# JamesBrofos/Stein

Measured on AMD Instinct MI355X. Metric: SVGD particle-updates/sec, higher is better.
Workload: dtype f32; 1 GPU; C3 bayesian-logreg-shaped synthetic block n=16384 d=256 fp32 (roofline config); n=16384, d=256, rows_per_rank=16384, optimizer=adagrad lr=1e-3 alpha=0.9, parallelism=single GPU

## Files before the change

stein_amd/csrc/stein_x3.hip:

```cpp

#include "stein_x3.h"

#include <stdlib.h>

#include "stein_x3_dev.h"
template <int KIND> struct SplitTraits { static constexpr int pexp = KIND == 2 ? PEXP_H2 : 0; };

#include <type_traits>

__device__ __forceinline__ int xswz(int row, int chunk) { return (chunk ^ ((row >> 2) & 3)) * 16; }

__device__ __forceinline__ u32 cvt_pk_bf16(float lo, float hi) {
  u32 r;
  asm("v_cvt_pk_bf16_f32 %0, %1, %2" : "=v"(r) : "v"(lo), "v"(hi));
  return r;
}

template <int KIND>
__device__ __forceinline__ void split_pair(float x, float y, u32 (&w)[3]) {
  if (KIND == 2) {
    w[0] = cvt_pk_f16(x, y);
    w[1] = cvt_pk_f16(f16_resid_lo(w[0], x), f16_resid_hi(w[0], y));
  } else {
    w[0] = cvt_pk_bf16(x, y);
  }
}


__device__ __forceinline__ void write_global_scales(float* __restrict__ sc, int dc, int sa, int pexp) {
  sc[4 * dc + 0] = pow2i(sa);
  sc[4 * dc + 1] = pow2i(1 - 2 * sa);
  sc[4 * dc + 2] = pow2i(-pexp);
}

__device__ __forceinline__ void make_scales_body(const u32* cmax, int dc, float* __restrict__ sc, int pexp, int enable,
                                                 u32* red) {
  const int t = threadIdx.x;
  if (t < 256) {
    u32 m = 0u;
    for (int c = t; c < dc; c += 256) {
      const u32 mg = load_fresh(cmax + c), mt = load_fresh(cmax + dc + c);
      const int sg = enable ? scale_exp(mg, 100) : 0, st = enable ? scale_exp(mt, 100) : 0;
      sc[c] = pow2i(sg);
      sc[dc + c] = pow2i(st);
      sc[2 * dc + c] = pow2i(-sg - pexp);
      sc[3 * dc + c] = pow2i(-st - pexp);
      m = max(m, mt);
    }
    red[t] = m;
  }
  __syncthreads();
  for (int o = 128; o > 0; o >>= 1) {
    if (t < o) red[t] = max(red[t], red[t + o]);
    __syncthreads();
  }
  if (t == 0) write_global_scales(sc, dc, enable ? scale_exp(red[0], 60) : 0, pexp);
}

template <typename TIN, bool V4>
__global__ __launch_bounds__(V4 ? 1024 : 256) void k_colmax(const TIN* __restrict__ X0, const TIN* __restrict__ X1, int n, int d,
                                                            u32* __restrict__ cmax0, int dc, int zbase, float* __restrict__ sc,
                                                            int pexp, HistSync* done) {
  const int z = blockIdx.z + zbase;
  constexpr int CW = V4 ? 4 : 1;
  constexpr int NW = V4 ? 16 : 4;
  __shared__ u32 red[256];
  const int t = threadIdx.x, cx = t & 63, ry = t >> 6;
  const TIN* const X[1] = {z ? X1 : X0};
  u32 m[1][CW];
  colmax_scan<TIN, V4, 1>(X, n, d, ((int)blockIdx.x * 64 + cx) * CW, (long)blockIdx.y * NW + ry, (long)gridDim.y * NW, m);
  colmax_commit<CW, 1>(m, cx, (int)blockIdx.x, d, red, cmax0 + (z ? dc : 0), dc);
  if (done) {
    __shared__ u32 s_last;
    asm volatile("s_waitcnt vmcnt(0)" ::: "memory");
    __syncthreads();
    if (t == 0) {
      const u32 id = (blockIdx.z * gridDim.y + blockIdx.y) * gridDim.x + blockIdx.x;
      s_last = tree_report_done(done->cm_leaf, &done->cm_top, id, gridDim.x * gridDim.y * gridDim.z) ? 1u : 0u;
    }
    __syncthreads();
    if (s_last) make_scales_body(cmax0, dc, sc, pexp, 1, red);
  }
}

__global__ __launch_bounds__(256) void k_make_scales(const u32* __restrict__ cmax, int dc, float* __restrict__ sc, int pexp,
                                                     int enable) {
  __shared__ u32 red[256];
  make_scales_body(cmax, dc, sc, pexp, enable, red);
}

constexpr int TP_WORDS = 64 * 32;
__device__ __forceinline__ int tp_index(int c, int p) { return c * 32 + ((((p >> 2) ^ (c >> 2)) & 7) << 2) + (p & 3); }
__device__ __forceinline__ int tp_pair(int t, int pass) { return 16 * pass + 4 * (t >> 6) + (((t >> 4) & 3) ^ ((t >> 2) & 2)); }

template <typename TIN>
__device__ __forceinline__ void load_row4(const TIN* __restrict__ X, int row, int col, int n, int d, int vec, float (&v)[4]) {
  if constexpr (std::is_same<TIN, float>::value) {
    if (vec) {
      const float4 x = (row < n && col < d) ? *reinterpret_cast<const float4*>(X + (size_t)row * d + col) : make_float4(0.f, 0.f, 0.f, 0.f);
      v[0] = x.x; v[1] = x.y; v[2] = x.z; v[3] = x.w;
      return;
    }
  }
#pragma unroll
  for (int q = 0; q < 4; ++q) v[q] = (row < n && col + q < d) ? elem_f32(X + (size_t)row * d + col + q) : 0.f;
}

template <int KIND>
__device__ __forceinline__ void tp_store(const u32 (*tile)[TP_WORDS], u16* __restrict__ Tt, long ntk_t, int dc, long nk,
                                         int row0, int col0, int t) {
  const int c = col0 + (t >> 2), j = row0 + (t & 3) * 16;
  if (c < dc && j < nk) {
    const int rowc = c & 127, ch0 = (j & 31) >> 3;
#pragma unroll
    for (int s = 0; s < KIND; ++s) {
      const uint4 w0 = *reinterpret_cast<const uint4*>(&tile[s][tp_index(t >> 2, (t & 3) * 8)]);
      const uint4 w1 = *reinterpret_cast<const uint4*>(&tile[s][tp_index(t >> 2, (t & 3) * 8 + 4)]);
      u16* base = Tt + (((size_t)(c >> 7) * ntk_t + (j >> 5)) * 3 + s) * XTILE_E;
      *reinterpret_cast<uint4*>(base + vfrag_offset(rowc, ch0)) = w0;
      *reinterpret_cast<uint4*>(base + vfrag_offset(rowc, ch0 + 1)) = w1;
    }
  }
}

template <typename TIN, int KIND, bool PRO = false>
__global__ __launch_bounds__(256) void k_split(const TIN* __restrict__ X0, const TIN* __restrict__ X1, int n, int d,
                                               u16* __restrict__ R0, long r_rows, int dk, u16* __restrict__ Tt0,
                                               u16* __restrict__ Tt1, int dc, long nk, const float* __restrict__ sc,
                                               int zbase, PrologueArgs pro, int vec) {
  if (PRO && blockIdx.z == gridDim.z - 1) {
    prologue_body<TIN>(X0, pro, (int)(blockIdx.y * gridDim.x + blockIdx.x), (int)(gridDim.x * gridDim.y));
    return;
  }
  const bool score = blockIdx.z + zbase != 0;
  if (score && ((int)blockIdx.x * 64 >= dc || (long)blockIdx.y * 64 >= nk)) return;
  const TIN* __restrict__ X = score ? X1 : X0;
  u16* __restrict__ R = score ? nullptr : R0;
  u16* __restrict__ Tt = score ? Tt1 : Tt0;
  const float* __restrict__ sc_all = sc + 4 * dc;
  const float* __restrict__ sc_col = sc + (score ? 0 : dc);
  __shared__ __attribute__((aligned(16))) u32 tile[KIND][TP_WORDS];
  const int t = threadIdx.x;
  const int row0 = blockIdx.y * 64, col0 = blockIdx.x * 64;
  const int lc = (t & 15) * 4;
  const long ntk_r = dk >> 5, ntk_t = nk >> 5;
  const float sa = (R && !PRO) ? *sc_all : 1.f;
  float scq[4];
#pragma unroll
  for (int q = 0; q < 4; ++q) scq[q] = (!PRO && Tt && col0 + lc + q < dc) ? sc_col[col0 + lc + q] : 1.f;
#pragma unroll
  for (int p = 0; p < 2; ++p) {
    const int pr = tp_pair(t, p), col = col0 + lc;
    float v[2][4];
#pragma unroll
    for (int h = 0; h < 2; ++h) {
      const int row = row0 + 2 * pr + h;
      load_row4(X, row, col, n, d, vec, v[h]);
      if (R && row < r_rows && col < dk) {
        u32 wa[3], wb[3];
        split_pair<KIND>(v[h][0] * sa, v[h][1] * sa, wa);
        split_pair<KIND>(v[h][2] * sa, v[h][3] * sa, wb);
        u16* dst = R + (((size_t)(row >> 7) * ntk_r + (col >> 5)) * 3) * XTILE_E + vfrag_offset(row & 127, (col & 31) >> 3) + (col & 7);
#pragma unroll
        for (int s = 0; s < KIND; ++s) *reinterpret_cast<uint2*>(dst + s * XTILE_E) = make_uint2(wa[s], wb[s]);
      }
    }
    if (Tt) {
#pragma unroll
      for (int q = 0; q < 4; ++q) {
        u32 w[3];
        split_pair<KIND>(v[0][q] * scq[q], v[1][q] * scq[q], w);
#pragma unroll
        for (int s = 0; s < KIND; ++s) tile[s][tp_index(lc + q, pr)] = w[s];
      }
    }
  }
  if (!Tt) return;
  __syncthreads();
  tp_store<KIND>(tile, Tt, ntk_t, dc, nk, row0, col0, t);
}

__global__ __launch_bounds__(256) void k_split_rows(const float* __restrict__ X, int n, int d, u16* __restrict__ R, long r_rows,
                                                    int dk, int dc, float* __restrict__ sc, int vec,
                                                    const u32* __restrict__ wgmax, int nwg) {
  __shared__ u32 s_wmax[4];
  const int t = threadIdx.x;
  const int row0 = blockIdx.y * 64, col = blockIdx.x * 64 + (t & 15) * 4;
  const long ntk_r = dk >> 5;
  u32 m = 0u;
  for (int i = t; i < nwg; i += 256) m = max(m, wgmax[i]);
  float v[2][2][4];
#pragma unroll
  for (int p = 0; p < 2; ++p)
#pragma unroll
    for (int h = 0; h < 2; ++h) load_row4(X, row0 + 2 * tp_pair(t, p) + h, col, n, d, vec, v[p][h]);
#pragma unroll
  for (int o = 32; o > 0; o >>= 1) m = max(m, (u32)__shfl_xor((int)m, o));
  if ((t & 63) == 0) s_wmax[t >> 6] = m;
  __syncthreads();
  const int sae = scale_exp(max(max(s_wmax[0], s_wmax[1]), max(s_wmax[2], s_wmax[3])), 60);
  const float sa = pow2i(sae);
  if (t == 0 && blockIdx.x == 0 && blockIdx.y == 0) write_global_scales(sc, dc, sae, PEXP_H2);
#pragma unroll
  for (int p = 0; p < 2; ++p)
#pragma unroll
    for (int h = 0; h < 2; ++h) {
      const int row = row0 + 2 * tp_pair(t, p) + h;
      if (row < r_rows && col < dk) {
        u32 wa[3], wb[3];
        split_pair<2>(v[p][h][0] * sa, v[p][h][1] * sa, wa);
        split_pair<2>(v[p][h][2] * sa, v[p][h][3] * sa, wb);
        u16* dst = R + (((size_t)(row >> 7) * ntk_r + (col >> 5)) * 3) * XTILE_E + vfrag_offset(row & 127, (col & 31) >> 3) + (col & 7);
#pragma unroll
        for (int s = 0; s < 2; ++s) *reinterpret_cast<uint2*>(dst + s * XTILE_E) = make_uint2(wa[s], wb[s]);
      }
    }
}

__global__ __launch_bounds__(256) void k_split_w(const float* __restrict__ T, const float* __restrict__ G, int n, int d,
                                                 u16* __restrict__ Wt, int dc, long nk, float* __restrict__ sc,
                                                 const u32* __restrict__ cmax, const float* __restrict__ h2p, int vec) {
  __shared__ __attribute__((aligned(16))) u32 tile[2][TP_WORDS];
  const int t = threadIdx.x;
  const int row0 = blockIdx.y * 64, col0 = blockIdx.x * 64;
  const int lc = (t & 15) * 4;
  const long ntk_t = nk >> 5;
  const float ih = 1.f / *h2p;
  float scq[4];
#pragma unroll
  for (int q = 0; q < 4; ++q) {
    const int c = col0 + lc + q;
    int se = 0;
    if (c < dc) se = scale_exp(__float_as_uint(__builtin_fmaf(__uint_as_float(cmax[dc + c]), ih, __uint_as_float(cmax[c]))), 100);
    scq[q] = pow2i(se);
    if (blockIdx.y == 0 && (t >> 4) == 0 && c < dc) {
      sc[c] = scq[q];
      sc[2 * dc + c] = pow2i(-se - PEXP_H2);
      const int st = scale_exp(cmax[dc + c], 100);
      sc[dc + c] = pow2i(st);
      sc[3 * dc + c] = pow2i(-st - PEXP_H2);
    }
  }
#pragma unroll
  for (int p = 0; p < 2; ++p) {
    const int pr = tp_pair(t, p), col = col0 + lc;
    float v[2][4];
#pragma unroll
    for (int h = 0; h < 2; ++h) {
      const int row = row0 + 2 * pr + h;
      float th[4], g[4];
      load_row4(T, row, col, n, d, vec, th);
      load_row4(G, row, col, n, d, vec, g);
#pragma unroll
      for (int q = 0; q < 4; ++q) v[h][q] = (row < n && col + q < d) ? __builtin_fmaf(-th[q], ih, g[q]) : 0.f;
    }
#pragma unroll
    for (int q = 0; q < 4; ++q) {
      u32 w[3];
      split_pair<2>(v[0][q] * scq[q], v[1][q] * scq[q], w);
#pragma unroll
      for (int s = 0; s < 2; ++s) tile[s][tp_index(lc + q, pr)] = w[s];
    }
  }
  __syncthreads();
  tp_store<2>(tile, Wt, ntk_t, dc, nk, row0, col0, t);
}

__device__ __forceinline__ const u16* t3_chunk_ptr(const u16* __restrict__ T3, long ntk, long grow, int c16) {
  return T3 + ((size_t)(grow >> 7) * ntk * 3) * XTILE_E + vfrag_offset((int)(grow & 127), c16);
}

template <int NP>
__device__ __forceinline__ void t3_load(const u16* __restrict__ p0, const u16* __restrict__ p1, int kt, u32x4 (&reg)[6]) {
#pragma unroll
  for (int s = 0; s < NP; ++s) {
    reg[s * 2 + 0] = *reinterpret_cast<const u32x4*>(p0 + ((size_t)kt * 3 + s) * XTILE_E);
    reg[s * 2 + 1] = *reinterpret_cast<const u32x4*>(p1 + ((size_t)kt * 3 + s) * XTILE_E);
  }
}

template <int NP>
__device__ __forceinline__ void x3_store_swz(unsigned char* oper, int t, const u32x4 (&reg)[6]) {
#pragma unroll
  for (int s = 0; s < NP; ++s)
#pragma unroll
    for (int q = 0; q < 2; ++q) {
      const int chunk = t + 256 * q;
      *reinterpret_cast<u32x4*>(oper + s * XPLANE + (chunk >> 2) * XROW + xswz(chunk >> 2, chunk & 3)) = reg[s * 2 + q];
    }
}

template <int NP>
__device__ __forceinline__ f32x16 x3_products(const u32x4 (&a)[3], const u32x4 (&b)[3], f32x16 c) {
  if (NP == 2) {
    c = __builtin_amdgcn_mfma_f32_32x32x16_f16(X3_HF(a[1]), X3_HF(b[0]), c, 0, 0, 0);
    c = __builtin_amdgcn_mfma_f32_32x32x16_f16(X3_HF(a[0]), X3_HF(b[1]), c, 0, 0, 0);
    return __builtin_amdgcn_mfma_f32_32x32x16_f16(X3_HF(a[0]), X3_HF(b[0]), c, 0, 0, 0);
  }
  return __builtin_amdgcn_mfma_f32_32x32x16_bf16(X3_BF(a[0]), X3_BF(b[0]), c, 0, 0, 0);
}


template <int NP>
__device__ __forceinline__ void x3_mma_tile(const unsigned char* As, const unsigned char* Bs, int wy, int wx, int lane,
                                            f32x16 (&acc)[2][2]) {
  const int l31 = lane & 31, h = lane >> 5;
#pragma unroll
  for (int ks = 0; ks < 2; ++ks) {
    u32x4 a[2][3], b[2][3];
    const int co = xswz(l31, 2 * ks + h);
#pragma unroll
    for (int i = 0; i < 2; ++i)
#pragma unroll
      for (int s = 0; s < NP; ++s) {
        a[i][s] = *reinterpret_cast<const u32x4*>(As + s * XPLANE + (wy * 64 + i * 32 + l31) * XROW + co);
        b[i][s] = *reinterpret_cast<const u32x4*>(Bs + s * XPLANE + (wx * 64 + i * 32 + l31) * XROW + co);
      }
#pragma unroll
    for (int i = 0; i < 2; ++i)
#pragma unroll
      for (int j = 0; j < 2; ++j) acc[i][j] = x3_products<NP>(a[i], b[j], acc[i][j]);
  }
}

template <bool SYM, int NP>
__global__ __launch_bounds__(NTHREADS, 3) void k_distance_x3(const u16* __restrict__ T3, int ntk,
                                                             const float* __restrict__ r, float* __restrict__ D, int n,
                                                             int row0, int n_local, long ldD, int tiles_m, int tiles_n,
                                                             u64* __restrict__ hist0, const float* __restrict__ two_s,
                                                             SpecState* __restrict__ spec, u64* __restrict__ spec_buf) {
  constexpr int OP = NP * XPLANE;
  __shared__ __attribute__((aligned(16))) unsigned char smem[2 * OP > EPI_LDS_BYTES ? 2 * OP : EPI_LDS_BYTES];
  unsigned char* As = smem;
  unsigned char* Bs = smem + OP;
  int tile_m, tile_n;
  if (!distance_tile<SYM>(xcd_remap(blockIdx.x, gridDim.x), tiles_m, tiles_n, tile_m, tile_n)) return;
  const int t = threadIdx.x, lane = t & 63, wid = t >> 6;
  const int wy = wid >> 1, wx = wid & 1;
  const long arow0 = row0 + (long)tile_m * BM, brow0 = (long)tile_n * BN;
  const EpiPrefetch pf = distance_epilogue_prefetch(r, n, row0, n_local, tile_m, tile_n, spec);
  const float two_s_v = *two_s;

  f32x16 acc[2][2];
#pragma unroll
  for (int i = 0; i < 2; ++i)
#pragma unroll
    for (int j = 0; j < 2; ++j)
#pragma unroll
      for (int e = 0; e < 16; ++e) acc[i][j][e] = 0.f;

  const u16* __restrict__ pa0 = t3_chunk_ptr(T3, ntk, arow0 + (t >> 2), t & 3);
  const u16* __restrict__ pa1 = t3_chunk_ptr(T3, ntk, arow0 + (t >> 2) + 64, t & 3);
  const u16* __restrict__ pb0 = t3_chunk_ptr(T3, ntk, brow0 + (t >> 2), t & 3);
  const u16* __restrict__ pb1 = t3_chunk_ptr(T3, ntk, brow0 + (t >> 2) + 64, t & 3);
  u32x4 ra[6], rb[6];
  t3_load<NP>(pa0, pa1, 0, ra);
  t3_load<NP>(pb0, pb1, 0, rb);
  for (int kt = 0; kt < ntk; ++kt) {
    x3_store_swz<NP>(As, t, ra);
    x3_store_swz<NP>(Bs, t, rb);
    __syncthreads();
    if (kt + 1 < ntk) {
      t3_load<NP>(pa0, pa1, kt + 1, ra);
      t3_load<NP>(pb0, pb1, kt + 1, rb);
    }
    x3_mma_tile<NP>(As, Bs, wy, wx, lane, acc);
    __syncthreads();
  }
  distance_epilogue<SYM, false>(acc, reinterpret_cast<u32*>(smem), D, n, n_local, ldD, tile_m, tile_n, hist0, pf,
                                two_s_v, spec, spec_buf);
}

constexpr int FS_THREADS = 768;

constexpr int FS_KT = 4;
constexpr int FS_ROWS = 128;
constexpr int FS_IB = FS_ROWS / 16;
constexpr int CJ = 2;
constexpr int PR = FS_ROWS / 32;
constexpr int PLN = FS_ROWS * XROW;

template <int NP, bool FOLD = false>
__global__ __launch_bounds__(FS_THREADS) void k_phi_x3fs(const float* __restrict__ D, long ldD,
                                                         const u16* __restrict__ Gt3, const u16* __restrict__ Tt3,
                                                         long ntj, const float* __restrict__ h2p,
                                                         float* __restrict__ OG, float* __restrict__ OT,
                                                         float* __restrict__ RS, int n, int d, int n_local,
                                                         int tiles_m, int cblocks, int split, int jchunk,
                                                         const float* __restrict__ sc, int dc, int upper) {
  const int wpm = FOLD ? (cblocks + 1) >> 1 : cblocks;
  constexpr int FS_KTB = NP * PLN;
  constexpr int FS_STAGE = FS_KT * FS_KTB;
  __shared__ __attribute__((aligned(16))) unsigned char smem[2 * FS_STAGE];

  const int logical = xcd_remap(blockIdx.x, gridDim.x);
  int cb, tile_m;
  const int plane = wpm * tiles_m;
  const int half = FOLD && logical >= plane * split ? 1 : 0;
  const int lw = FOLD ? logical - half * plane * split : logical;
  const int l2 = lw % plane;
  const int z = lw / plane;
  if (wpm > 4 && (wpm & 3) == 0 && (tiles_m & 7) == 0) {
    const int sb = l2 >> 5, in = l2 & 31, cgroups = wpm >> 2;
    cb = (sb % cgroups) * 4 + (in & 3);
    tile_m = (sb / cgroups) * 8 + (in >> 2);
  } else {
    cb = l2 % wpm;
    tile_m = l2 / wpm;
  }
  const int i0 = tile_m * FS_ROWS;
  const int jbeg = z * jchunk;
  const int jend = half ? n : min(n, jbeg + jchunk);
  const int ntile = jend > jbeg ? (jend - jbeg + BK - 1) / BK : 0;
  const int nstage = (ntile + FS_KT - 1) / FS_KT;
  const int rot = (cb % FS_KT) * (wpm >= FS_KT ? 1 : FS_KT / wpm) % FS_KT;
  const int group = wpm <= 32 ? 32 / wpm : 1;
  const bool permute = upper != 0 && (FOLD || (jbeg == 0 && jend == n && nstage == tiles_m)) && (wpm & (wpm - 1)) == 0 &&
                       wpm <= 4 && nstage * FS_KT == ntile && (nstage & (nstage - 1)) == 0 && nstage >= 2 * group;
  const int xmask = permute ? (tile_m & ~(group - 1) & (nstage - 1)) : 0;
  auto stage_of = [&](int v) { return v ^ xmask; };
  auto tile_at = [&](int stage, int u) {
    const int st2 = stage_of(stage + u / FS_KT), u2 = u % FS_KT;
    return st2 * FS_KT + ((st2 + 1) * FS_KT <= ntile ? ((u2 + rot) & (FS_KT - 1)) : u2);
  };

  const bool up = upper != 0;
  const int ntr = up ? max(0, min(nstage, (i0 - jbeg) / (FS_KT * BK))) : 0;

  const int t = threadIdx.x;
  if (t < 256) {
    const int pt = t;
    const int lr = pt >> 3, lc = (pt & 7) * 4;
    float rs[PR];
#pragma unroll
    for (int p = 0; p < PR; ++p) rs[p] = 0.f;
    constexpr int PD = FOLD ? 2 : FS_KT;
    f32x4g rd[PD][PR];
    u32 doff[PR];
    const float cexp = -1.44269504088896341f / (2.f * *h2p);
    constexpr float pofs = (float)SplitTraits<NP>::pexp;
#pragma unroll
    for (int p = 0; p < PR; ++p) doff[p] = (u32)(((i0 & (DT_ROWS - 1)) + lr + 32 * p) * DT_COLS + lc);
    const float* __restrict__ drow = D + (size_t)(i0 / DT_ROWS) * (ldD >> 5) * DT_ELEMS;
    const int jq = (pt >> 3) & 7, ig = (pt >> 6) * 8 + (pt & 7);
    u32 doff_tr[PR];
#pragma unroll
    for (int u = 0; u < PR; ++u) doff_tr[u] = (u32)((ig >> 3) * DT_ELEMS + (4 * jq + u) * DT_COLS + 4 * (ig & 7)) * 4u;
    const long ntc_d = ldD >> 5;
    float rst[4] = {0.f, 0.f, 0.f, 0.f};
    auto request = [&](int j0, bool tr, f32x4g (&rd)[PR]) {
      const float* tile = tr ? D + ((size_t)(j0 >> 7) * ntc_d + 4 * (size_t)(i0 / DT_ROWS)) * DT_ELEMS + (j0 & 127) * DT_COLS
                             : drow + (size_t)(j0 >> 5) * DT_ELEMS;
#pragma unroll
      for (int p = 0; p < PR; ++p) stream_load16(rd[p], tile, tr ? doff_tr[p] : doff[p] * 4u);
    };
    auto wait_loads = [&](int v, f32x4g (&rd)[PR]) {
      const int later = ntile - v - 1;
      (void)rd;
      if constexpr (PD == 4) {
        stream_wait<3 * PR>();
        if (later < 3) {
          stream_wait<2 * PR>();
          if (later < 2) {
            stream_wait<PR>();
            if (later < 1) stream_wait<0>();
          }
        }
      } else {
        static_assert(PD == 2 || PD == 4, "wait_loads is written out for these two leads");
        stream_wait<PR>();
        if (later < 1) stream_wait<0>();
      }
    };
    auto produce = [&](int j0, unsigned char* buf, const f32x4g (&rd)[PR]) {
      const bool full = j0 + BK <= jend;
      float q[PR][4];
#pragma unroll
      for (int p = 0; p < PR; ++p)
#pragma unroll
        for (int e = 0; e < 4; ++e) q[p][e] = __builtin_fmaf(cexp, rd[p][e], pofs);
      __builtin_amdgcn_sched_barrier(0);
#pragma unroll
      for (int p = 0; p < PR; ++p)
#pragma unroll
        for (int e = 0; e < 4; ++e) q[p][e] = __builtin_amdgcn_exp2f(q[p][e]);
      __builtin_amdgcn_sched_barrier(0);
      if (!full) {
        const int j = j0 + lc;
#pragma unroll
        for (int p = 0; p < PR; ++p)
#pragma unroll
          for (int e = 0; e < 4; ++e) q[p][e] = (j + e < jend) ? q[p][e] : 0.f;
      }
      if (NP >= 2) {
        u32 hi[PR][2], lo[PR][2];
        float r[PR][4];
#pragma unroll
        for (int p = 0; p < PR; ++p) rs[p] += (q[p][0] + q[p][1]) + (q[p][2] + q[p][3]);
#pragma unroll
        for (int p = 0; p < PR; ++p) { hi[p][0] = cvt_pk_f16(q[p][0], q[p][1]); hi[p][1] = cvt_pk_f16(q[p][2], q[p][3]); }
        __builtin_amdgcn_sched_barrier(0);
#pragma unroll
        for (int p = 0; p < PR; ++p) {
          r[p][0] = f16_resid_lo(hi[p][0], q[p][0]); r[p][1] = f16_resid_hi(hi[p][0], q[p][1]);
          r[p][2] = f16_resid_lo(hi[p][1], q[p][2]); r[p][3] = f16_resid_hi(hi[p][1], q[p][3]);
        }
        __builtin_amdgcn_sched_barrier(0);
#pragma unroll
        for (int p = 0; p < PR; ++p) { lo[p][0] = cvt_pk_f16(r[p][0], r[p][1]); lo[p][1] = cvt_pk_f16(r[p][2], r[p][3]); }
        __builtin_amdgcn_sched_barrier(0);
#pragma unroll
        for (int p = 0; p < PR; ++p) {
          unsigned char* dst = buf + (lr + 32 * p) * XROW + pswz(lr, lc >> 3) + (lc & 4) * 2;
          *reinterpret_cast<uint2*>(dst) = make_uint2(hi[p][0], hi[p][1]);
          *reinterpret_cast<uint2*>(dst + PLN) = make_uint2(lo[p][0], lo[p][1]);
        }
      } else {
#pragma unroll
        for (int p = 0; p < PR; ++p) {
          unsigned char* dst = buf + (lr + 32 * p) * XROW + pswz(lr, lc >> 3) + (lc & 4) * 2;
          const u32 h0 = cvt_pk_bf16(q[p][0], q[p][1]), h1 = cvt_pk_bf16(q[p][2], q[p][3]);
          rs[p] += (__uint_as_float(h0 << 16) + __uint_as_float(h0 & 0xffff0000u)) +
                   (__uint_as_float(h1 << 16) + __uint_as_float(h1 & 0xffff0000u));
          *reinterpret_cast<uint2*>(dst) = make_uint2(h0, h1);
        }
      }
    };
    auto produce_tr = [&](unsigned char* buf, const f32x4g (&rd)[PR]) {
      float q[4][4];
#pragma unroll
      for (int u = 0; u < 4; ++u)
#pragma unroll
        for (int e = 0; e < 4; ++e) q[u][e] = __builtin_fmaf(cexp, rd[u][e], pofs);
      __builtin_amdgcn_sched_barrier(0);
#pragma unroll
      for (int u = 0; u < 4; ++u)
#pragma unroll
        for (int e = 0; e < 4; ++e) q[u][e] = __builtin_amdgcn_exp2f(q[u][e]);
      __builtin_amdgcn_sched_barrier(0);
      u32 hi[4][2], lo[4][2];
      if (NP >= 2) {
        float r[4][4];
#pragma unroll
        for (int e = 0; e < 4; ++e) rst[e] += (q[0][e] + q[1][e]) + (q[2][e] + q[3][e]);
#pragma unroll
        for (int e = 0; e < 4; ++e) { hi[e][0] = cvt_pk_f16(q[0][e], q[1][e]); hi[e][1] = cvt_pk_f16(q[2][e], q[3][e]); }
        __builtin_amdgcn_sched_barrier(0);
#pragma unroll
        for (int e = 0; e < 4; ++e) {
          r[e][0] = f16_resid_lo(hi[e][0], q[0][e]); r[e][1] = f16_resid_hi(hi[e][0], q[1][e]);
          r[e][2] = f16_resid_lo(hi[e][1], q[2][e]); r[e][3] = f16_resid_hi(hi[e][1], q[3][e]);
        }
        __builtin_amdgcn_sched_barrier(0);
#pragma unroll
        for (int e = 0; e < 4; ++e) { lo[e][0] = cvt_pk_f16(r[e][0], r[e][1]); lo[e][1] = cvt_pk_f16(r[e][2], r[e][3]); }
        __builtin_amdgcn_sched_barrier(0);
      } else {
#pragma unroll
        for (int e = 0; e < 4; ++e) {
          hi[e][0] = cvt_pk_bf16(q[0][e], q[1][e]); hi[e][1] = cvt_pk_bf16(q[2][e], q[3][e]);
          lo[e][0] = lo[e][1] = 0u;
          rst[e] += (__uint_as_float(hi[e][0] << 16) + __uint_as_float(hi[e][0] & 0xffff0000u)) +
                    (__uint_as_float(hi[e][1] << 16) + __uint_as_float(hi[e][1] & 0xffff0000u));
        }
      }
#pragma unroll
      for (int e = 0; e < 4; ++e) {
        const int row = 4 * ig + e;
        unsigned char* dst = buf + row * XROW + pswz(row, jq >> 1) + (jq & 1) * 8;
        *reinterpret_cast<uint2*>(dst) = make_uint2(hi[e][0], hi[e][1]);
        if (NP >= 2) *reinterpret_cast<uint2*>(dst + PLN) = make_uint2(lo[e][0], lo[e][1]);
      }
    };
    auto jt = [&](int tile) { return jbeg + tile * BK; };
#pragma unroll
    for (int u = 0; u < PD; ++u)
      if (tile_at(0, u) < ntile) request(jt(tile_at(0, u)), stage_of(0) < ntr, rd[u]);
    auto produce_stage = [&](int st, unsigned char* buf) {
      const bool tr_now = stage_of(st) < ntr;
#pragma unroll
      for (int u = 0; u < FS_KT; ++u) {
        const int tile_u = tile_at(st, u), next_u = tile_at(st, u + PD);
        const bool tr_next = stage_of(st + (u + PD) / FS_KT) < ntr;
        if (tile_u < ntile) {
          wait_loads(st * FS_KT + u, rd[u % PD]);
          if (tr_now) produce_tr(buf + u * FS_KTB, rd[u % PD]);
          else produce(jt(tile_u), buf + u * FS_KTB, rd[u % PD]);
        }
        if (next_u < ntile) request(jt(next_u), tr_next, rd[u % PD]);
      }
    };
    produce_stage(0, smem);
    __syncthreads();
    for (int st = 0; st < nstage; ++st) {
      if (st + 1 < nstage) produce_stage(st + 1, smem + ((st + 1) & 1) * FS_STAGE);
      __syncthreads();
    }
    if (up) {
      float* red = reinterpret_cast<float*>(smem);
#pragma unroll
      for (int p = 0; p < 4; ++p) {
        float a = rs[p], b = rst[p];
        a += __shfl_xor(a, 1); b += __shfl_xor(b, 8);
        a += __shfl_xor(a, 2); b += __shfl_xor(b, 16);
        a += __shfl_xor(a, 4); b += __shfl_xor(b, 32);
        if ((pt & 7) == 0) red[lr + 32 * p] = a;
        if (jq == 0) red[128 + 4 * ig + p] = b;
      }
      __syncthreads();
      const int row = i0 + pt;
      if (cb == 0 && !half && pt < 128 && row < n_local) RS[(size_t)z * n_local + row] = (red[pt] + red[128 + pt]) * sc[4 * dc + 2];
    } else if (cb == 0 && !half) {
#pragma unroll
      for (int p = 0; p < PR; ++p) {
        float sum = rs[p];
        sum += __shfl_xor(sum, 1);
        sum += __shfl_xor(sum, 2);
        sum += __shfl_xor(sum, 4);
        const int row = i0 + lr + 32 * p;
        if ((pt & 7) == 0 && row < n_local) RS[(size_t)z * n_local + row] = sum * sc[4 * dc + 2];
      }
    }
  } else {
    const int ct = t - 256, lane = ct & 63, cw = ct >> 6;
    const int l15 = lane & 15, lq = lane >> 4;
    const int g = 2 * cb + (cw >> 2);
    const int gl = FOLD ? min(g, cblocks - 1) : g;
    const int wcol = (cw & 3) * 32;
    const u16* vb_wave = (FOLD ? (half ? Tt3 : Gt3) + (size_t)gl * ntj * 3 * XTILE_E
                               : (g < cblocks ? Gt3 + (size_t)g * ntj * 3 * XTILE_E
                                              : Tt3 + (size_t)(g - cblocks) * ntj * 3 * XTILE_E)) +
                         (size_t)(jbeg >> 5) * 3 * XTILE_E + wcol * 32;
    const u16* __restrict__ vb = reinterpret_cast<const u16*>(
        ((unsigned long long)(u32)__builtin_amdgcn_readfirstlane((int)((unsigned long long)vb_wave >> 32)) << 32) |
        (unsigned long long)(u32)__builtin_amdgcn_readfirstlane((int)(unsigned long long)vb_wave));
    u32 boff[CJ][3];
#pragma unroll
    for (int j = 0; j < CJ; ++j)
#pragma unroll
      for (int s = 0; s < 3; ++s) boff[j][s] = (u32)(lane * 8 + s * XTILE_E + j * 512) * 2u;
    const int aoff = l15 * XROW + pswz(l15, lq);
    f32x4 acc[FS_IB][CJ];
#pragma unroll
    for (int i = 0; i < FS_IB; ++i)
#pragma unroll
      for (int j = 0; j < CJ; ++j) acc[i][j] = f32x4{0.f, 0.f, 0.f, 0.f};
    u32x4 bX[CJ][3], bY[CJ][3];
    auto load_b = [&](int tile, u32x4 (&b)[CJ][3]) {
      const u16* __restrict__ src = vb + (size_t)tile * 3 * XTILE_E;
#pragma unroll
      for (int j = 0; j < CJ; ++j)
#pragma unroll
        for (int s = 0; s < NP; ++s) stream_load16(b[j][s], src, boff[j][s]);
    };
    auto wait_b = [&](bool younger, u32x4 (&b)[CJ][3]) {
      (void)b;
      stream_wait<CJ * NP>();
      if (!younger) stream_wait<0>();
    };
    auto read_a = [&](const unsigned char* As, int i, u32x4 (&a)[3]) {
#pragma unroll
      for (int s = 0; s < NP; ++s) a[s] = *reinterpret_cast<const u32x4*>(As + aoff + i * 16 * XROW + s * PLN);
    };
    auto mma_tile = [&](const unsigned char* As, const u32x4 (&b)[CJ][3]) {
      u32x4 a[2][3];
      read_a(As, 0, a[0]);
#pragma unroll
      for (int i = 0; i < FS_IB; ++i) {
        if (i + 1 < FS_IB) read_a(As, i + 1, a[(i + 1) & 1]);
        __builtin_amdgcn_sched_barrier(0);
#pragma unroll
        for (int j = 0; j < CJ; ++j) acc[i][j] = x3_products16<NP>(a[i & 1], b[j], acc[i][j]);
        __builtin_amdgcn_sched_barrier(0);
      }
    };
    if (ntile > 0) load_b(tile_at(0, 0), bX);
    __syncthreads();
    for (int st = 0; st < nstage; ++st) {
      const unsigned char* As = smem + (st & 1) * FS_STAGE;
      auto after = [&](int u) { return tile_at(st, u); };
      constexpr bool kLoadV = true;
#pragma unroll
      for (int u = 0; u < FS_KT; u += 2) {
        if (after(u) >= ntile) break;
        const bool n1 = after(u + 1) < ntile;
        if (kLoadV && n1) load_b(after(u + 1), bY);
        wait_b(kLoadV && n1, bX);
        if (cw >> 2) __builtin_amdgcn_s_setprio(0); else __builtin_amdgcn_s_setprio(2);
        mma_tile(As + u * FS_KTB, bX);
        if (n1) {
          const bool n2 = after(u + 2) < ntile;
          if (kLoadV && n2) load_b(after(u + 2), bX);
          wait_b(kLoadV && n2, bY);
          if (cw >> 2) __builtin_amdgcn_s_setprio(2); else __builtin_amdgcn_s_setprio(0);
          mma_tile(As + (u + 1) * FS_KTB, bY);
        }
      }
      __syncthreads();
    }
    if (up) __syncthreads();
    if (FOLD ? g >= cblocks : g >= 2 * cblocks) return;
    const bool first = FOLD ? half == 0 : g < cblocks;
    float* __restrict__ Oz = (first ? OG : OT) + (size_t)z * n_local * d;
    const int cbase = (FOLD || first ? g : g - cblocks) * BN + wcol + l15;
    const float* __restrict__ osc = sc + (first ? 2 : 3) * dc;
#pragma unroll
    for (int j = 0; j < CJ; ++j) {
      const int col = cbase + j * 16;
      if (col >= d) continue;
      const float os = osc[col];
#pragma unroll
      for (int i = 0; i < FS_IB; ++i)
#pragma unroll
        for (int e = 0; e < 4; ++e) {
          const int row = i0 + i * 16 + 4 * lq + e;
          if (row < n_local) Oz[(size_t)row * d + col] = acc[i][j][e] * os;
        }
    }
  }
}

static int split_kind(int dtype) { return dtype == STEIN_BF16 ? 1 : 2; }
int stein_x3_kind(int dtype) { return split_kind(dtype); }

template <typename TIN, int KIND>
static void launch_split(hipStream_t stream, const TIN* theta, const TIN* score, int64_t n, int64_t d,
                         const SteinLayout& L, u16* T3, u16* Tt3, u16* Gt3, const float* sc, const PrologueArgs* pro = nullptr) {
  const unsigned nz = (theta ? 1u : 0u) + (score ? 1u : 0u);
  const int zbase = theta ? 0 : 1;
  const int vec = std::is_same<TIN, float>::value && d % 4 == 0 && (((uintptr_t)theta | (uintptr_t)score) & 15u) == 0;
  const int64_t rows = L.x3_rows > L.x3_nk ? L.x3_rows : L.x3_nk;
  const int64_t cols = L.x3_dk > L.x3_dc ? L.x3_dk : L.x3_dc;
  if (KIND == 1 && pro && theta) {
    const dim3 grid((unsigned)((cols + 63) / 64), (unsigned)((rows + 63) / 64), nz + 1u);
    hipLaunchKernelGGL((k_split<TIN, KIND, true>), grid, dim3(256), 0, stream, theta, score, (int)n, (int)d, T3,
                       (long)L.x3_rows, (int)L.x3_dk, Tt3, Gt3, (int)L.x3_dc, (long)L.x3_nk, sc, zbase, *pro, vec);
    return;
  }
  const dim3 grid((unsigned)((cols + 63) / 64), (unsigned)((rows + 63) / 64), nz);
  hipLaunchKernelGGL((k_split<TIN, KIND, false>), grid, dim3(256), 0, stream, theta, score, (int)n, (int)d, T3,
                     (long)L.x3_rows, (int)L.x3_dk, Tt3, Gt3, (int)L.x3_dc, (long)L.x3_nk, sc, zbase, PrologueArgs{}, vec);
}

static void launch_colmax(const StepViews& v, const float* score_all, const float* theta_all, int64_t n, int64_t d,
                          HistSync* fuse_done, hipStream_t stream) {
  const int dc = (int)v.L.x3_dc;
  const int zbase = score_all ? 0 : 1;
  const unsigned nz = (score_all ? 1u : 0u) + (theta_all ? 1u : 0u);
  int gy = (int)((n + 63) / 64);
  if (gy > 256) gy = 256;
  const bool v4 = d % 4 == 0 && (!score_all || ((uintptr_t)score_all & 15) == 0) && (!theta_all || ((uintptr_t)theta_all & 15) == 0);
  if (v4) {
    const int gy4 = gy > 64 ? 64 : gy;
    const dim3 grid((unsigned)((d + 255) / 256), (unsigned)gy4, nz);
    hipLaunchKernelGGL((k_colmax<float, true>), grid, dim3(1024), 0, stream, score_all, theta_all, (int)n, (int)d, v.cmax, dc,
                       zbase, v.sc, PEXP_H2, fuse_done);
  } else {
    const dim3 grid((unsigned)((d + 63) / 64), (unsigned)gy, nz);
    hipLaunchKernelGGL((k_colmax<float, false>), grid, dim3(256), 0, stream, score_all, theta_all, (int)n, (int)d, v.cmax, dc,
                       zbase, v.sc, PEXP_H2, fuse_done);
  }
}

int stein_x3_split(const StepViews& v, const void* theta_all, const void* score_all, int dtype, int64_t n, int64_t d,
                   hipStream_t stream, const SplitFused* fused) {
  const SteinLayout& L = v.L;
  const int dc = (int)L.x3_dc;
  const int kind = split_kind(dtype);
  HistSync* fuse_done = fused && theta_all && score_all ? fused->done : nullptr;
  const PrologueArgs* prologue = fused ? fused->prologue : nullptr;
  const int fold = fused ? fused->fold : 0;
  const u32* wgmax = fused && kind == 2 && fold == 1 ? fused->wgmax : nullptr;
  if (wgmax) {
    const int vec = d % 4 == 0 && ((uintptr_t)theta_all & 15u) == 0;
    const dim3 grid((unsigned)((L.x3_dk + 63) / 64), (unsigned)((L.x3_rows + 63) / 64));
    hipLaunchKernelGGL(k_split_rows, grid, dim3(256), 0, stream, (const float*)theta_all, (int)n, (int)d, v.T3, (long)L.x3_rows,
                       (int)L.x3_dk, dc, v.sc, vec, wgmax, fused->nwg);
    LAUNCH_CHECK("k_split_rows");
    return STEIN_OK;
  }
  if (kind == 2) {
    const int zbase = score_all ? 0 : 1;
    const unsigned nz = (score_all ? 1u : 0u) + (theta_all ? 1u : 0u);
    if (!fuse_done) HIP_TRY(hipMemsetAsync(v.cmax + (size_t)zbase * dc, 0, (size_t)nz * dc * sizeof(u32), stream));
    launch_colmax(v, (const float*)score_all, (const float*)theta_all, n, d, fuse_done, stream);
    LAUNCH_CHECK("k_colmax");
  }
  if (kind == 2 ? !fuse_done : !prologue) {
    hipLaunchKernelGGL(k_make_scales, dim3(1), dim3(256), 0, stream, v.cmax, dc, v.sc, kind == 2 ? PEXP_H2 : 0,
                       kind == 2 ? 1 : 0);
    LAUNCH_CHECK("k_make_scales");
  }
  if (kind == 1) launch_split<u16, 1>(stream, (const u16*)theta_all, (const u16*)score_all, n, d, L, v.T3, v.Tt3, v.Gt3, v.sc, prologue);
  else if (fold)
    launch_split<float, 2>(stream, (const float*)theta_all, (const float*)nullptr, n, d, L, v.T3, fold == 2 ? v.Tt3 : nullptr, v.Gt3, v.sc);
  else launch_split<float, 2>(stream, (const float*)theta_all, (const float*)score_all, n, d, L, v.T3, v.Tt3, v.Gt3, v.sc);
  LAUNCH_CHECK("k_split");
  return STEIN_OK;
}

constexpr double FOLD_MIN_WORK = 4.0e9;
bool stein_fold_pays(int64_t n, int64_t d) { return d > 128 && (double)n * (double)n * (double)d >= FOLD_MIN_WORK; }

int stein_x3_colmax(const StepViews& v, const float* theta_all, const float* score_all, int64_t n, int64_t d,
                    hipStream_t stream) {
  launch_colmax(v, score_all, theta_all, n, d, nullptr, stream);
  LAUNCH_CHECK("k_colmax");
  return STEIN_OK;
}

int stein_x3_split_w(const StepViews& v, const float* theta_all, const float* score_all, int64_t n, int64_t d,
                     const float* h2_dev, hipStream_t stream) {
  const SteinLayout& L = v.L;
  const dim3 grid((unsigned)((L.x3_dc + 63) / 64), (unsigned)((L.x3_nk + 63) / 64));
  const int vec = d % 4 == 0 && (((uintptr_t)theta_all | (uintptr_t)score_all) & 15u) == 0;
  hipLaunchKernelGGL(k_split_w, grid, dim3(256), 0, stream, theta_all, score_all, (int)n, (int)d, v.Gt3, (int)L.x3_dc,
                     (long)L.x3_nk, v.sc, (const u32*)v.cmax, h2_dev, vec);
  LAUNCH_CHECK("k_split_w");
  return STEIN_OK;
}

template <bool SYM, int NP>
static void launch_distance_x3(long nblk, hipStream_t stream, const u16* T3, int ntk, const float* r, float* D, int n,
                               int row0, int n_local, long ld, int tiles_m, int tiles_n, u64* hist0, const float* two_s,
                               SpecState* spec, u64* spec_buf) {
  hipLaunchKernelGGL((k_distance_x3<SYM, NP>), dim3((unsigned)nblk), dim3(NTHREADS), 0, stream, T3, ntk, r, D, n, row0,
                     n_local, ld, tiles_m, tiles_n, hist0, two_s, spec, spec_buf);
}

int stein_x3_distance(const StepViews& v, const BlockShape& b, bool symmetric, bool window, hipStream_t stream, int panel) {
  if (panel >= 0 && stein_dpanel_ok(v, b, panel > 0)) return stein_dpanel_distance(v, b, symmetric, window, stream);
  const SteinLayout& L = v.L;
  const int ntk = (int)(L.x3_dk / 32);
  const int tiles_m = (int)((b.n_local + BM - 1) / BM), tiles_n = (int)((b.n + BN - 1) / BN);
  if (b.row0 + (int64_t)tiles_m * BM > L.x3_rows) return stein_fail(STEIN_E_SHAPE, "row block exceeds the padded planes");
  const long nblk = distance_grid(symmetric, tiles_m, tiles_n);
  if (nblk > 0x7fffffffl) return stein_fail(STEIN_E_SHAPE, "too many tiles");
  SpecState* spec = window ? v.spec : nullptr;
  u64* spec_buf = window ? v.spec_buf : nullptr;
#define X3_DIST(SYM, NP) launch_distance_x3<SYM, NP>(nblk, stream, v.T3, ntk, v.r, v.D, (int)b.n, (int)b.row0, (int)b.n_local, (long)L.ld_dist, tiles_m, tiles_n, v.hist, v.two_s, spec, spec_buf)
  switch (split_kind(b.dtype)) {
    case 1: if (symmetric) X3_DIST(true, 1); else X3_DIST(false, 1); break;
    default: if (symmetric) X3_DIST(true, 2); else X3_DIST(false, 2); break;
  }
#undef X3_DIST
  LAUNCH_CHECK("k_distance_x3");
  return STEIN_OK;
}

int stein_x3_contract_partial(const StepViews& v, const BlockShape& b, const float* h2_dev, hipStream_t stream, bool upper) {
  const SteinLayout& L = v.L;
  const long nblk = (long)L.tiles_m * L.cblocks * v.nsplit;
  if (nblk > 0x7fffffffl) return stein_fail(STEIN_E_SHAPE, "too many tiles");
#define X3_PHI(NP) hipLaunchKernelGGL((k_phi_x3fs<NP>), dim3((unsigned)nblk), dim3(FS_THREADS), 0, stream, v.D, (long)L.ld_dist, v.Gt3, v.Tt3, (long)(L.x3_nk / 32), h2_dev, v.OG, v.OT, v.RS, (int)b.n, (int)b.d, (int)b.n_local, (int)L.tiles_m, (int)L.cblocks, v.nsplit, v.jchunk, v.sc, (int)L.x3_dc, upper ? 1 : 0)
  switch (split_kind(b.dtype)) {
    case 1: X3_PHI(1); break;
    default: X3_PHI(2); break;
  }
#undef X3_PHI
  LAUNCH_CHECK("k_phi_x3fs");
  return STEIN_OK;
}

int stein_x3_contract_fold(const StepViews& v, const float* h2_dev, int64_t n, int64_t d, bool with_theta,
                           hipStream_t stream) {
  const SteinLayout& L = v.L;
  const long per_range = (long)L.tiles_m * ((L.cblocks + 1) / 2);
  const long nblk = per_range * (v.nsplit + (with_theta ? 1 : 0));
  if (nblk > 0x7fffffffl) return stein_fail(STEIN_E_SHAPE, "too many tiles");
  hipLaunchKernelGGL((k_phi_x3fs<2, true>), dim3((unsigned)nblk), dim3(FS_THREADS), 0, stream, v.D, (long)L.ld_dist, v.Gt3,
                     with_theta ? v.Tt3 : (const u16*)nullptr, (long)(L.x3_nk / 32), h2_dev, v.OG, v.OT, v.RS, (int)n, (int)d,
                     (int)n, (int)L.tiles_m, (int)L.cblocks, v.nsplit, v.jchunk, v.sc, (int)L.x3_dc, 1);
  LAUNCH_CHECK("k_phi_x3fs");
  return STEIN_OK;
}
```

Before: 27.07 million particle-updates/s.

## Stage phi kernel output through LDS image for coalesced vectorized global stores

The MFMA accumulator epilogue now writes scaled results into a swizzled shared-memory image that reuses the stage buffers, instead of issuing scattered per-element global stores. All 12 waves, producer waves included, then read the image and write rows to OG/OT as 16-byte vectors, with a scalar fallback when alignment does not allow it. When NP is not 2 the work runs in two passes. The row-sum reduction scratch moves to an extra 1KB of LDS so it does not collide with the image. The aim is to cut uncoalesced write traffic in the epilogue, at the cost of added barriers, more LDS use, and more epilogue work on every thread.

```diff
diff --git a/stein_amd/csrc/stein_x3.hip b/stein_amd/csrc/stein_x3.hip
--- a/stein_amd/csrc/stein_x3.hip
+++ b/stein_amd/csrc/stein_x3.hip
@@ -391,7 +391,7 @@
   const int wpm = FOLD ? (cblocks + 1) >> 1 : cblocks;
   constexpr int FS_KTB = NP * PLN;
   constexpr int FS_STAGE = FS_KT * FS_KTB;
-  __shared__ __attribute__((aligned(16))) unsigned char smem[2 * FS_STAGE];
+  __shared__ __attribute__((aligned(16))) unsigned char smem[2 * FS_STAGE + 1024];
 
   const int logical = xcd_remap(blockIdx.x, gridDim.x);
   int cb, tile_m;
@@ -428,6 +428,58 @@
   const int ntr = up ? max(0, min(nstage, (i0 - jbeg) / (FS_KT * BK))) : 0;
 
   const int t = threadIdx.x;
+  constexpr int IMG_COLS = NP == 2 ? 256 : 128;
+  constexpr int IMG_PITCH = IMG_COLS * 16;
+  constexpr int IMG_PASSES = 256 / IMG_COLS;
+  static_assert(32 * IMG_PITCH <= 2 * FS_STAGE, "the output image lives in the stage buffers");
+  const bool vec16 = (d & 3) == 0 && ((((size_t)OG) | ((size_t)OT)) & 15) == 0;
+  auto image_store = [&](int ps) {
+    const int wv = __builtin_amdgcn_readfirstlane(t >> 6), ln = t & 63;
+    if (vec16) {
+      constexpr int MB = IMG_COLS / 32, NT = 4 * MB;
+#pragma unroll
+      for (int q = 0; q < (NT + 11) / 12; ++q) {
+        const int task = wv + 12 * q;
+        if (task >= NT) break;
+        const int mb = task % MB, rg = (task / MB) * 8 + (ln >> 3);
+        const int g = 2 * cb + (NP == 2 ? mb >> 2 : ps);
+        if (FOLD && g >= cblocks) continue;
+        const bool first = FOLD ? half == 0 : g < cblocks;
+        float* __restrict__ Oz = (first ? OG : OT) + (size_t)z * n_local * d;
+        const int c = 32 * mb + 4 * (ln & 7);
+        const int col = (FOLD || first ? g : g - cblocks) * BN + (c & (BN - 1));
+        const int row = i0 + 4 * rg;
+        if (col < d && row < n_local) {
+          const unsigned char* src = smem + rg * IMG_PITCH;
+          f32x4 u[4];
+#pragma unroll
+          for (int k = 0; k < 4; ++k) u[k] = *reinterpret_cast<const f32x4*>(src + (((c + k) ^ (rg & 3)) * 16));
+#pragma unroll
+          for (int e = 0; e < 4; ++e)
+            if (row + e < n_local)
+              *reinterpret_cast<f32x4*>(Oz + (size_t)(row + e) * d + col) = f32x4{u[0][e], u[1][e], u[2][e], u[3][e]};
+        }
+      }
+    } else {
+      constexpr int CH = IMG_COLS / 64, NI = 32 * CH;
+      for (int item = wv; item < NI; item += 12) {
+        const int ch = item % CH, rg = item / CH;
+        const int g = 2 * cb + (NP == 2 ? ch >> 1 : ps);
+        if (FOLD && g >= cblocks) continue;
+        const bool first = FOLD ? half == 0 : g < cblocks;
+        float* __restrict__ Oz = (first ? OG : OT) + (size_t)z * n_local * d;
+        const int c = 64 * ch + ln;
+        const int col = (FOLD || first ? g : g - cblocks) * BN + (c & (BN - 1));
+        const int row = i0 + 4 * rg;
+        if (col < d && row < n_local) {
+          const f32x4 u = *reinterpret_cast<const f32x4*>(smem + rg * IMG_PITCH + ((c ^ (rg & 3)) * 16));
+#pragma unroll
+          for (int e = 0; e < 4; ++e)
+            if (row + e < n_local) Oz[(size_t)(row + e) * d + col] = u[e];
+        }
+      }
+    }
+  };
   if (t < 256) {
     const int pt = t;
     const int lr = pt >> 3, lc = (pt & 7) * 4;
@@ -597,7 +649,7 @@
       __syncthreads();
     }
     if (up) {
-      float* red = reinterpret_cast<float*>(smem);
+      float* red = reinterpret_cast<float*>(smem + 2 * FS_STAGE);
 #pragma unroll
       for (int p = 0; p < 4; ++p) {
         float a = rs[p], b = rst[p];
@@ -607,9 +659,6 @@
         if ((pt & 7) == 0) red[lr + 32 * p] = a;
         if (jq == 0) red[128 + 4 * ig + p] = b;
       }
-      __syncthreads();
-      const int row = i0 + pt;
-      if (cb == 0 && !half && pt < 128 && row < n_local) RS[(size_t)z * n_local + row] = (red[pt] + red[128 + pt]) * sc[4 * dc + 2];
     } else if (cb == 0 && !half) {
 #pragma unroll
       for (int p = 0; p < PR; ++p) {
@@ -620,6 +669,18 @@
         const int row = i0 + lr + 32 * p;
         if ((pt & 7) == 0 && row < n_local) RS[(size_t)z * n_local + row] = sum * sc[4 * dc + 2];
       }
+    }
+    __syncthreads();
+    if (up) {
+      const float* red = reinterpret_cast<const float*>(smem + 2 * FS_STAGE);
+      const int row = i0 + pt;
+      if (cb == 0 && !half && pt < 128 && row < n_local) RS[(size_t)z * n_local + row] = (red[pt] + red[128 + pt]) * sc[4 * dc + 2];
+    }
+    image_store(0);
+    if (IMG_PASSES == 2) {
+      __syncthreads();
+      __syncthreads();
+      image_store(1);
     }
   } else {
     const int ct = t - 256, lane = ct & 63, cw = ct >> 6;
@@ -698,24 +759,34 @@
       }
       __syncthreads();
     }
-    if (up) __syncthreads();
-    if (FOLD ? g >= cblocks : g >= 2 * cblocks) return;
     const bool first = FOLD ? half == 0 : g < cblocks;
-    float* __restrict__ Oz = (first ? OG : OT) + (size_t)z * n_local * d;
     const int cbase = (FOLD || first ? g : g - cblocks) * BN + wcol + l15;
     const float* __restrict__ osc = sc + (first ? 2 : 3) * dc;
-#pragma unroll
-    for (int j = 0; j < CJ; ++j) {
-      const int col = cbase + j * 16;
-      if (col >= d) continue;
-      const float os = osc[col];
-#pragma unroll
-      for (int i = 0; i < FS_IB; ++i)
-#pragma unroll
-        for (int e = 0; e < 4; ++e) {
-          const int row = i0 + i * 16 + 4 * lq + e;
-          if (row < n_local) Oz[(size_t)row * d + col] = acc[i][j][e] * os;
-        }
+    unsigned char* const img = smem + lq * IMG_PITCH + ((((NP == 2 ? (cw >> 2) * BN : 0) + wcol + l15) ^ lq) * 16);
+    auto image_write = [&]() {
+      if (FOLD ? g >= cblocks : g >= 2 * cblocks) return;
+#pragma unroll
+      for (int j = 0; j < CJ; ++j) {
+        const int col = cbase + j * 16;
+        if (col >= d) continue;
+        const float os = osc[col];
+#pragma unroll
+        for (int i = 0; i < FS_IB; ++i) {
+          f32x4 v;
+#pragma unroll
+          for (int e = 0; e < 4; ++e) v[e] = acc[i][j][e] * os;
+          *reinterpret_cast<f32x4*>(img + i * 4 * IMG_PITCH + j * 16 * 16) = v;
+        }
+      }
+    };
+    if (NP == 2 || (cw >> 2) == 0) image_write();
+    __syncthreads();
+    image_store(0);
+    if (IMG_PASSES == 2) {
+      __syncthreads();
+      if ((cw >> 2) == 1) image_write();
+      __syncthreads();
+      image_store(1);
     }
   }
 }
```

After: 27.46 million particle-updates/s (median of 6 runs). 1.5% higher.
